# auduno/headtrackr

Measured on NVIDIA H100. Metric: frames/sec @640x480 (detect+CAMShift), higher is better.
Workload: dtype u8+f64

## Files before the change

headtrackr_b200/_lib.py:

```python
import ctypes as C
import os
import shutil
import subprocess
from pathlib import Path

_PKG = Path(__file__).resolve().parent
SO_PATH = Path(os.environ["HT_LIB"]).resolve() if os.environ.get("HT_LIB") else _PKG / "libheadtrackr_b200.so"
CSRC = _PKG / "csrc"

HT_OK, HT_WARN_OVERFLOW = 0, 1
HT_ERR_ARG, HT_ERR_CUDA, HT_ERR_SIZE, HT_ERR_CASCADE, HT_ERR_STATE = -1, -2, -3, -4, -5


class HtError(RuntimeError):
    def __init__(self, code, msg):
        super().__init__(f"headtrackr_b200 error {code}: {msg}")
        self.code = code


class Rect(C.Structure):
    _fields_ = [("x", C.c_double), ("y", C.c_double), ("width", C.c_double), ("height", C.c_double),
                ("confidence", C.c_double), ("neighbors", C.c_int32), ("pad_", C.c_int32)]


# ... 128 lines not shown
                ("cuda_stream", C.c_void_p)]


def sources_newer_than_so():
    if not SO_PATH.exists():
        return True
    t = SO_PATH.stat().st_mtime
    srcs = list(CSRC.glob("*.cu")) + list(CSRC.glob("*.cuh")) + list(CSRC.glob("*.inc")) + \
        [_PKG.parent / "include" / "headtrackr_b200.h"]
    return any(s.stat().st_mtime > t for s in srcs)


def nvcc():
    home = os.environ.get("CUDA_HOME") or os.environ.get("CUDA_PATH")
    if home and (Path(home) / "bin" / "nvcc").exists():
        return str(Path(home) / "bin" / "nvcc")
    return shutil.which("nvcc") or "/usr/local/cuda/bin/nvcc"


def build(force=False):
    if force or sources_newer_than_so():
        subprocess.check_call(["make", "-s", "-C", str(CSRC), f"NVCC={nvcc()}"] + (["-B"] if force else []))
    if not SO_PATH.exists():
        raise ImportError(f"{SO_PATH} was not produced by the build")
    return SO_PATH


_lib = None

EXPORTS = ["ht_version", "ht_create", "ht_destroy", "ht_last_error", "ht_sync", "ht_max_rects", "ht_detect",
           "ht_track_init", "ht_track_init_from_detect", "ht_track", "ht_detect_track", "ht_stream_reset", "ht_stream_step", "ht_stream_head_config", "ht_stream_step_head",
           "ht_tracker_config", "ht_tracker_reset", "ht_tracker_start", "ht_tracker_stop", "ht_tracker_step", "ht_tracker_feed", "ht_tracker_set_params", "ht_tracker_feed_canvases", "ht_tracker_set_debug", "ht_tracker_set_debug_strokes", "ht_tracker_set_face_crop", "ht_tracker_set_face_crop_yuv", "ht_tracker_set_face_tensor", "ht_face_crop_map", "ht_tracker_set_camera", "ht_tracker_export", "ht_tracker_import", "ht_tracker_feed_yuv", "ht_ingest", "ht_ingest_yuv",
           "ht_tracker_feed_views", "ht_tracker_feed_yuv_views", "ht_ingest_views", "ht_ingest_yuv_views", "ht_backprojection", "ht_whitebalance",
           "ht_plan_info", "ht_debug_plane", "ht_debug_raw", "ht_debug_model_hist", "ht_debug_track_stats", "ht_set_track_memo", "ht_set_pipeline", "ht_join", "ht_debug_set_exactness", "ht_debug_track_trace", "ht_debug_track_phases", "ht_launch_count",
           "ht_profile", "ht_profile_read"]

PROF_CLASSES = ["gray", "pyramid", "cascade", "group", "hist", "track_init", "track"]


def lib():
    global _lib
    if _lib is not None:
        return _lib
    if not SO_PATH.exists():
        try:
            build()
        except Exception as e:
            raise ImportError(f"libheadtrackr_b200.so is missing and could not be built: {e}") from e
    L = C.CDLL(str(SO_PATH))
    vp = C.c_void_p
    L.ht_version.restype = C.c_uint32
    L.ht_create.argtypes = [C.POINTER(vp), C.POINTER(Config), C.c_char_p, C.c_size_t]
    L.ht_destroy.argtypes = [vp]
    L.ht_destroy.restype = None
    L.ht_last_error.argtypes = [vp]
    L.ht_last_error.restype = C.c_char_p
    L.ht_sync.argtypes = [vp]
    L.ht_max_rects.argtypes = [vp]
    L.ht_detect.argtypes = [vp, vp, C.c_int, C.c_int, C.c_int, C.c_int, C.c_int, vp, vp]
    L.ht_track_init.argtypes = [vp, vp, C.c_int, vp, C.c_int, C.c_int, vp, C.c_int]
    L.ht_track_init_from_detect.argtypes = [vp, vp, C.c_int, vp, C.c_int, C.c_int, vp, vp, C.c_int, vp]
    L.ht_track.argtypes = [vp, vp, C.c_int, vp, C.c_int, C.c_int, C.c_int, vp, vp]
    L.ht_detect_track.argtypes = [vp, vp, C.c_int, C.c_int, C.c_int, C.c_int, C.c_int, C.c_int, C.c_int,
                                  vp, vp, vp, vp, vp]
    L.ht_stream_reset.argtypes = [vp, C.c_int, C.c_int]
    L.ht_stream_step.argtypes = [vp, vp, C.c_int, C.c_int, C.c_int, C.c_int, C.c_int, C.c_int, vp]
    L.ht_stream_head_config.argtypes = [vp, vp]
    L.ht_stream_step_head.argtypes = [vp, vp, C.c_int, C.c_int, C.c_int, C.c_int, C.c_int, C.c_int, vp, vp]
    L.ht_tracker_config.argtypes = [vp, vp]
    for f in (L.ht_tracker_reset, L.ht_tracker_start, L.ht_tracker_stop):
        f.argtypes = [vp, C.c_int, C.c_int]
    L.ht_tracker_step.argtypes = [vp, vp, C.c_int, C.c_int, C.c_int, C.c_double, vp]
    L.ht_tracker_feed.argtypes = [vp, vp, C.c_int, C.c_int, C.c_int, C.c_int, vp]
    L.ht_tracker_set_params.argtypes = [vp, C.c_int, C.c_int, vp]
    L.ht_tracker_feed_canvases.argtypes = [vp, vp, C.c_int, C.c_int, vp]
    L.ht_tracker_set_debug.argtypes = [vp, C.c_int, C.c_int, vp]
    L.ht_tracker_set_debug_strokes.argtypes = [vp, C.c_int, C.c_int, vp]
    L.ht_tracker_set_face_crop.argtypes = [vp, C.c_int, C.c_int, vp]
    L.ht_tracker_set_face_crop_yuv.argtypes = [vp, C.c_int, C.c_int, vp]
    L.ht_tracker_set_face_tensor.argtypes = [vp, C.c_int, C.c_int, vp]
    L.ht_face_crop_map.argtypes = [vp, C.c_int, C.c_int, C.c_int, C.c_int, vp, vp, vp]
    L.ht_tracker_set_camera.argtypes = [vp, C.c_int, C.c_int, vp]
    L.ht_tracker_export.argtypes = [vp, vp, C.c_int, vp]
    L.ht_tracker_import.argtypes = [vp, vp, C.c_int, vp]
    L.ht_ingest.argtypes = [vp, vp, C.c_int, C.c_int, C.c_int, vp, C.c_int, C.c_int]
    L.ht_tracker_feed_yuv.argtypes = [vp, vp, C.c_int, C.c_int, vp]
    L.ht_ingest_yuv.argtypes = [vp, vp, C.c_int, C.c_int, vp, C.c_int, C.c_int]
    L.ht_tracker_feed_views.argtypes = [vp, vp, vp, C.c_int, C.c_int, vp]
    L.ht_tracker_feed_yuv_views.argtypes = [vp, vp, vp, C.c_int, C.c_int, vp]
    L.ht_ingest_views.argtypes = [vp, vp, vp, C.c_int, C.c_int, vp, C.c_int, C.c_int]
    L.ht_ingest_yuv_views.argtypes = [vp, vp, vp, C.c_int, C.c_int, vp, C.c_int, C.c_int]
    L.ht_backprojection.argtypes = [vp, C.c_int, vp, C.c_int, C.c_int, vp]
    L.ht_whitebalance.argtypes = [vp, vp, C.c_int, C.c_int, C.c_int, vp]
    L.ht_plan_info.argtypes = [vp, C.c_int, C.c_int, C.c_int, vp, vp, vp, vp, C.c_int]
    L.ht_debug_plane.argtypes = [vp, C.c_int, C.c_int, C.c_int, vp, C.c_int, vp, vp]
    L.ht_debug_raw.argtypes = [vp, C.c_int, vp, C.c_int, vp]
    L.ht_debug_model_hist.argtypes = [vp, C.c_int, vp]
    L.ht_debug_track_stats.argtypes = [vp, vp, C.c_int]
    L.ht_debug_track_trace.argtypes = [vp, vp, C.c_int]
    L.ht_debug_track_phases.argtypes = [vp, vp, C.c_int]
    L.ht_set_track_memo.argtypes = [vp, C.c_int]
    L.ht_set_pipeline.argtypes = [vp, C.c_int]
    L.ht_join.argtypes = [vp]
    L.ht_debug_set_exactness.argtypes = [vp, C.c_int]
    L.ht_launch_count.argtypes = [vp]
    L.ht_launch_count.restype = C.c_uint64
    L.ht_profile.argtypes = [vp, C.c_int]
    L.ht_profile_read.argtypes = [vp, vp, vp, C.c_int]
    _lib = L
    return L
```

headtrackr_b200/context.py:

```python
import ctypes as C
import math

import numpy as np

from . import _lib
from ._lib import (Camera, CameraControl, CanvasFrame, DebugCanvas, FaceCrop, FaceCropYuv, FaceTensor, HeadEvent, HeadParams, HtError, Rect, StreamEvent, TrackerEvent, TrackerParams, TrackObj, VideoFrame,
                   VideoView, Window, YuvFrame, YuvImage)
from .views import video_view
from .synth import load_cascade_blob


def _is_torch(x):
    return hasattr(x, "data_ptr") and hasattr(x, "is_cuda")


def _frames_ptr(frames):
    if _is_torch(frames):
        t = frames
        if t.dim() == 3:
            t = t.unsqueeze(0)
        if not t.is_contiguous() or t.element_size() != 1 or t.shape[-1] != 4:
            raise ValueError("frames tensor must be contiguous uint8 (n,H,W,4)")
        return t.data_ptr(), t.shape[0], t.shape[1], t.shape[2], t
    a = np.ascontiguousarray(frames, dtype=np.uint8)
# ... 720 lines not shown
        cnt = C.c_int32()
        self._check(self._L.ht_debug_raw(self._h, frame, C.addressof(out), cap, C.addressof(cnt)))
        kept = min(cnt.value, cap, self.raw_cap)
        return [(r.x, r.y, r.width, r.height, r.confidence, r.neighbors) for r in out[:kept]], cnt.value

    def debug_track_stats(self, reset=True):
        out = (C.c_uint64 * 5)()
        self._check(self._L.ht_debug_track_stats(self._h, C.addressof(out), int(bool(reset))))
        return dict(passes=int(out[0]), serial_passes=int(out[1]), pixels=int(out[2]), calls=int(out[3]),
                    memo_hits=int(out[4]))

    def set_track_memo(self, enable=True):
        self._check(self._L.ht_set_track_memo(self._h, int(bool(enable))))

    def set_pipeline(self, enable=True):
        self._check(self._L.ht_set_pipeline(self._h, int(bool(enable))))

    def join(self):
        self._check(self._L.ht_join(self._h))

    def debug_set_exactness(self, flags):
        self._check(self._L.ht_debug_set_exactness(self._h, int(flags)))

    def debug_track_trace(self, n):
        out = np.zeros((n, 4), np.uint64)
        self._check(self._L.ht_debug_track_trace(self._h, out.ctypes.data, n))
        return out

    def debug_track_phases(self, n):
        out = np.zeros((n, 8), np.uint64)
        self._check(self._L.ht_debug_track_phases(self._h, out.ctypes.data, n))
        return out

    def debug_model_hist(self, slot):
        out = np.zeros(4096, np.uint32)
        self._check(self._L.ht_debug_model_hist(self._h, slot, out.ctypes.data))
        return out


def tracker_params(retryDetection=True, calcAngles=False, smoothing=True, fov=None, cameraOffset=11.5, headPosition=True,
                   edgecorrection=True, alpha=0.35, distance_to_screen=60.0):
    head = HeadParams(int(bool(smoothing)), int(bool(headPosition)), int(bool(edgecorrection)), 0, alpha,
                      float(fov) if fov is not None else 0.0, cameraOffset, distance_to_screen)
    return TrackerParams(int(bool(retryDetection)), int(bool(calcAngles)), (C.c_int32 * 2)(), head)


def tracker_event_dict(e):
    return dict(detection=("", "VJ", "CS", "WB")[e.detection], x=e.x, y=e.y, width=e.width, height=e.height,
                angle=e.angle, confidence=e.confidence, wb=e.wb, running=bool(e.running), fov=e.fov,
                status=[s for b, s in enumerate(_lib.TRACKER_STATUS) if e.status >> b & 1],
                head=dict(valid=bool(e.head.valid), x=e.head.x, y=e.head.y, z=e.head.z,
                          face=(e.head.fx, e.head.fy, e.head.fwidth, e.head.fheight)))


def tracker_events_from_bytes(buf):
    n = len(buf) // C.sizeof(TrackerEvent)
    arr = (TrackerEvent * n).from_buffer_copy(bytes(buf[: n * C.sizeof(TrackerEvent)]))
    return [tracker_event_dict(e) for e in arr]
```

headtrackr_b200/csrc/ht_api.cu:

```cuda
#include "../../include/headtrackr_b200.h"

#include <cuda.h>
#include <cuda_runtime.h>

#include <algorithm>
#include <cassert>
#include <cmath>
#include <cstdarg>
#include <cstddef>
#include <cstdio>
#include <cstdlib>
#include <cstring>
#include <map>
#include <memory>
#include <string>
#include <tuple>
#include <utility>
#include <vector>

#include "ht_common.cuh"
#include "ht_detect.cuh"
#include "ht_track.cuh"

using namespace ht;
// ... 320 lines not shown
    int g = 0;
    const int cuts_fast[] = {0, 2, 3, 4, 6};
    const int cuts_int[] = {0, 2, 4, 6};
    const int cuts_fp[] = {0, 2, 4, 6, 9};
    static_assert(HT_GEN_STAGES == 8, "cuts_fast assumes 8 generated stages");
    if (hc.fast) {
      for (int cpos : cuts_fast) cc.group_first[g++] = cpos;
      cc.group_first[g] = HT_GEN_STAGES;
      cc.late_int = 1;
    } else if (ints_ok && !getenv("HT_NO_LATE")) {
      for (int cpos : cuts_int) if (cpos < hc.n_stages) cc.group_first[g++] = cpos;
      cc.group_first[g] = std::min(8, hc.n_stages);
      cc.late_int = 1;
    } else {
      for (int cpos : cuts_fp) if (cpos < hc.n_stages) cc.group_first[g++] = cpos;
      cc.group_first[g] = hc.n_stages;
      cc.late_int = 0;
    }
    cc.n_groups = g;
  }
  hc.late.clear();
  hc.late_chunk0.assign((size_t)hc.n_stages + 1, 0);
  hc.late_conflicts = 0;
  for (int j = 0; j < hc.n_stages; ++j) {
    hc.late_chunk0[j] = (int32_t)(hc.late.size() / 32);
    if (j < cc.group_first[cc.n_groups]) continue;
    std::vector<int> rem;
    for (int k = cc.stage[j].first; k < cc.stage[j].first + cc.stage[j].count; ++k) rem.push_back(k);
    std::stable_sort(rem.begin(), rem.end(), [&](int x, int y) {
      const int sx = (cc.np_nn[x] & 15) + (cc.np_nn[x] >> 4), sy = (cc.np_nn[y] & 15) + (cc.np_nn[y] >> 4);
      return sx > sy;
    });
    while (!rem.empty()) {
      int bank_word[10][32];
      for (auto &row : bank_word) for (int &v : row) v = -1;
      auto place_side = [&](int k, int side, uint16_t *out, bool allow_conflicts, bool dry) -> int {
        const int cnt = side ? (cc.np_nn[k] >> 4) : (cc.np_nn[k] & 15);
        const uint16_t *pt = &cc.off[k][side ? 5 : 0];
        int order[5] = {0, 1, 2, 3, 4}, best_cost = 1 << 30, best[5] = {0, 1, 2, 3, 4};
        do {
          int cost = 0;
          for (int i = 0; i < cnt; ++i) {
            const int slot = side * 5 + order[i], word = pt[i] & 0x7fff, bw = bank_word[slot][word & 31];
            if (bw >= 0 && bw != word) cost += 1 << 10;
            cost += order[i];
          }
          if (cost < best_cost) { best_cost = cost; for (int i = 0; i < 5; ++i) best[i] = order[i]; }
        } while (std::next_permutation(order, order + 5));
        const int conflicts = best_cost >> 10;
        if (conflicts && !allow_conflicts) return -1;
        if (!dry) {
          for (int i = 0; i < cnt; ++i) {
            const int slot = side * 5 + best[i], word = pt[i] & 0x7fff;
            if (bank_word[slot][word & 31] < 0) bank_word[slot][word & 31] = word;
            out[slot] = pt[i];
          }
        }
        return conflicts;
      };
      for (int lane = 0; lane < 32; ++lane) {
        struct { uint16_t off[10]; int32_t a_int; } lf;
        for (int q = 0; q < 10; ++q) lf.off[q] = 0xFFFF;
        lf.a_int = 0;
        if (!rem.empty()) {
          size_t pick = rem.size();
          for (size_t i = 0; i < rem.size() && pick == rem.size(); ++i)
            if (place_side(rem[i], 0, lf.off, false, true) == 0 && place_side(rem[i], 1, lf.off, false, true) == 0) pick = i;
          if (pick == rem.size()) {
            int best_c = 1 << 30;
            for (size_t i = 0; i < rem.size(); ++i) {
              const int cfl = place_side(rem[i], 0, lf.off, true, true) + place_side(rem[i], 1, lf.off, true, true);
              if (cfl < best_c) { best_c = cfl; pick = i; }
            }
          }
          const int k = rem[pick];
          hc.late_conflicts += place_side(k, 0, lf.off, true, false) + place_side(k, 1, lf.off, true, false);
          lf.a_int = (int32_t)a_int[k];
          rem.erase(rem.begin() + (long)pick);
        }
        LateFeat rec{};
        for (int q = 0; q < 10; ++q) rec.off[q] = late_encode(lf.off[q]);
        rec.a_int = lf.a_int;
        hc.late.push_back(rec);
      }
    }
  }
  hc.late_chunk0[hc.n_stages] = (int32_t)(hc.late.size() / 32);
// ... 2672 lines not shown
int ht_join(ht_ctx *ctx) {
  if (!ctx) return HT_ERR_ARG;
  return join_aux(ctx);
}

int ht_debug_track_stats(ht_ctx *ctx, uint64_t *out5, int reset) {
  if (!ctx || !out5) return HT_ERR_ARG;
  CK(cudaSetDevice(ctx->cfg.device));
  CK(cudaStreamSynchronize(ctx->stream));
  CK(cudaMemcpy(out5, ctx->d_flags.as<unsigned long long>() + 8, 5 * sizeof(uint64_t), cudaMemcpyDeviceToHost));
  if (reset) CK(cudaMemset(ctx->d_flags.as<unsigned long long>() + 8, 0, 5 * sizeof(uint64_t)));
  return HT_OK;
}

int ht_debug_track_trace(ht_ctx *ctx, uint64_t *out, int n) {
  if (!ctx || !out) return HT_ERR_ARG;
  if (!ctx->track_trace || !ctx->d_trace.p || n < 0 || n > ctx->cfg.max_frames)
    return ctx->fail(HT_ERR_ARG, "track timeline is not enabled (HT_TRACK_TRACE=1 at ht_create) or n is out of range");
  CK(cudaSetDevice(ctx->cfg.device));
  CK(cudaStreamSynchronize(ctx->stream));
  CK(cudaMemcpy(out, ctx->d_trace.p, 4 * sizeof(uint64_t) * (size_t)n, cudaMemcpyDeviceToHost));
  return HT_OK;
}

int ht_debug_track_phases(ht_ctx *ctx, uint64_t *out, int n) {
  if (!ctx) return HT_ERR_ARG;
  { const int jr = join_aux(ctx); if (jr != HT_OK) return jr; }
  if (!ctx->track_trace || !ctx->d_trace.p || n < 0 || n > ctx->cfg.max_frames)
    return ctx->fail(HT_ERR_ARG, "no track trace (create the context with HT_TRACK_TRACE=1)");
  CK(cudaSetDevice(ctx->cfg.device));
  CK(cudaStreamSynchronize(ctx->stream));
  CK(cudaMemcpy(out, ctx->d_trace.as<unsigned long long>() + 4 * (size_t)ctx->cfg.max_frames, 8 * sizeof(uint64_t) * (size_t)n, cudaMemcpyDeviceToHost));
  return HT_OK;
}

int ht_debug_model_hist(ht_ctx *ctx, int slot, uint32_t *out4096) {
  if (!ctx) return HT_ERR_ARG;
  { const int jr = join_aux(ctx); if (jr != HT_OK) return jr; }
  if (!out4096 || slot < 0 || slot >= ctx->cfg.max_frames || !ctx->model_hist.p) return ctx->fail(HT_ERR_ARG, "bad slot");
  CK(cudaSetDevice(ctx->cfg.device));
  CK(cudaStreamSynchronize(ctx->stream));
  CK(cudaMemcpy(out4096, ctx->model_hist.as<uint32_t>() + (size_t)slot * 4096, 4096 * sizeof(uint32_t), cudaMemcpyDeviceToHost));
  return HT_OK;
}

}

#ifdef HT_HOST_SELFTEST
extern "C" int ht_selftest_planes(int w, int h, int interval, int32_t *out, int cap) {
  Plan P;
  std::string err;
  if (build_plan(P, w, h, interval, 24, 24, err, false) != HT_OK) return -1;
  if ((int)P.planes.size() * 6 + 2 > cap) return -2;
  out[0] = (int32_t)P.planes.size();
  out[1] = (int32_t)P.arena_stride;
  for (size_t i = 0; i < P.planes.size(); ++i) {
    int slot = -1, q = -1;
    for (size_t k = 0; k < P.plane_id.size(); ++k) if (P.plane_id[k] == (int)i) { slot = (int)(k / 4); q = (int)(k % 4); }
    int32_t *o = out + 2 + 6 * i;
    o[0] = (int32_t)P.planes[i].off; o[1] = P.planes[i].pitch; o[2] = P.planes[i].w; o[3] = P.planes[i].h; o[4] = slot; o[5] = q;
  }
  return 0;
}

extern "C" int ht_selftest_head(const ht_head_params *params, int n, const double *cs , int camw,
                                int camh, ht_head_event *out) {
// ... 504 lines not shown
      }
  }
  for (int f = 0; f < 4; ++f) {
    std::sort(hits[f].begin(), hits[f].end(), [](const Hit &a, const Hit &b) { return a.key < b.key; });
    counts[f] = (int32_t)hits[f].size();
    for (size_t i = 0; i < hits[f].size() && (int)i < cap; ++i) {
      double *o = out + ((size_t)f * cap + i) * 4;
      o[0] = hits[f][i].x; o[1] = hits[f][i].y; o[2] = hits[f][i].width; o[3] = hits[f][i].conf;
    }
  }
  return 0;
}

int main(int argc, char **argv) {
  if (argc < 2) { fprintf(stderr, "usage: %s cascade.bin\n", argv[0]); return 2; }
  FILE *f = fopen(argv[1], "rb");
  if (!f) { perror("open"); return 2; }
  std::vector<uint8_t> blob;
  uint8_t buf[4096];
  size_t got;
  while ((got = fread(buf, 1, sizeof(buf), f)) > 0) blob.insert(blob.end(), buf, buf + got);
  fclose(f);
  HostCascade hc;
  std::string err;
  const int rc = parse_cascade(blob.data(), blob.size(), hc, err);
  if (rc != HT_OK) { fprintf(stderr, "parse_cascade: %s\n", err.c_str()); return 1; }
  const ConstCascade &cc = hc.cc;
  const int late_first = cc.group_first[cc.n_groups];
  long long bad = 0, used_slots = 0, used_instr = 0, conflicts = 0;
  for (int j = late_first; j < hc.n_stages; ++j) {
    std::vector<int> seen((size_t)cc.stage[j].count, 0);
    for (int ch = hc.late_chunk0[j]; ch < hc.late_chunk0[j + 1]; ++ch) {
      for (int s = 0; s < 10; ++s) {
        int bank_word[32];
        for (int &v : bank_word) v = -1;
        bool any = false;
        for (int lane = 0; lane < 32; ++lane) {
          const uint16_t o = late_decode(hc.late[(size_t)ch * 32 + lane].off[s]);
          if (o == 0xFFFF) continue;
          any = true; ++used_slots;
          const int word = o & 0x7fff;
          if (bank_word[word & 31] >= 0 && bank_word[word & 31] != word) ++conflicts;
          bank_word[word & 31] = word;
        }
        used_instr += any ? 1 : 0;
      }
      for (int lane = 0; lane < 32; ++lane) {
        const LateFeat &lf = hc.late[(size_t)ch * 32 + lane];
        std::vector<uint16_t> p, n;
        for (int s = 0; s < 5; ++s) if (lf.off[s] != LATE_UNUSED) p.push_back(late_decode(lf.off[s]));
        for (int s = 5; s < 10; ++s) if (lf.off[s] != LATE_UNUSED) n.push_back(late_decode(lf.off[s]));
        if (p.empty() && n.empty()) { if (lf.a_int != 0) ++bad; continue; }
        std::sort(p.begin(), p.end()); std::sort(n.begin(), n.end());
        int match = -1;
        for (int k = cc.stage[j].first; k < cc.stage[j].first + cc.stage[j].count && match < 0; ++k) {
          if (seen[(size_t)(k - cc.stage[j].first)]) continue;
          std::vector<uint16_t> kp(cc.off[k], cc.off[k] + (cc.np_nn[k] & 15)), kn(cc.off[k] + 5, cc.off[k] + 5 + (cc.np_nn[k] >> 4));
          std::sort(kp.begin(), kp.end()); std::sort(kn.begin(), kn.end());
          if (kp == p && kn == n && llround(cc.alpha[k] * 1e8) == lf.a_int) match = k;
        }
        if (match < 0) ++bad; else seen[(size_t)(match - cc.stage[j].first)] = 1;
      }
    }
    for (int v : seen) if (!v) ++bad;
  }
  printf("{\"n_stages\": %d, \"n_features\": %d, \"fast\": %d, \"n_groups\": %d, \"late_first\": %d, \"chunks\": %d, "
         "\"bad\": %lld, \"point_loads\": %lld, \"load_instr_with_traffic\": %lld, \"bank_conflicts\": %lld, \"late_conflicts\": %d}\n",
         hc.n_stages, hc.n_features, hc.fast ? 1 : 0, cc.n_groups, late_first, hc.late_chunk0[hc.n_stages], bad, used_slots,
         used_instr, conflicts, hc.late_conflicts);
  return bad ? 1 : 0;
}
#endif
```

headtrackr_b200/csrc/ht_common.cuh:

```cuda
#pragma once
#include <cstddef>
#include <cstdint>

namespace ht {

constexpr int TW = 32;
constexpr int TH = 8;
constexpr int NV = 2 * TH;
constexpr int L0_COLS = 4 * TW + 22;
constexpr int L0_ROWS = 4 * TH + 22;
constexpr int H0 = L0_COLS / 2;
constexpr int P0 = L0_COLS;
constexpr int L1_ROWS = 2 * TH + 11;
constexpr int L1_COLS = 2 * TW + 11;
constexpr int P1 = 76;
constexpr int L2_ROWS = TH + 5;
constexpr int L2_COLS = TW + 5;
constexpr int P2 = 76;
constexpr int W1 = (L0_ROWS * P0 + 31) / 32 * 32;
constexpr int W2 = W1 + L1_ROWS * P1;
constexpr int TILE_WORDS = W2 + 2 * L2_ROWS * P2;
__host__ __device__ constexpr int tile_l0(int r, int X) { return r * P0 + (X & 1) * H0 + (X >> 1); }
__host__ __device__ constexpr int tile_l1(int r, int c) { return W1 + r * P1 + c; }
__host__ __device__ constexpr int tile_l2(int rr, int c2) { return W2 + rr * P2 + c2; }
constexpr int VA = 2 * P0;
constexpr int VB = P1;
static_assert((VA - VB) % 32 == 0 && P1 == P2, "bank classes of the two bases must coincide");
static_assert(2 * L2_COLS <= P2 && L1_COLS <= P1, "tile pitches");
constexpr int BANK_K = VA % 32;
static_assert(VB % 32 == BANK_K, "bank_class");
constexpr int NWIN = TW * TH * 4 * 4;
constexpr int MASK_WORDS = NV / 4;
static_assert(NV % 4 == 0, "TH must be even");
constexpr int CASCADE_THREADS = 256;
constexpr int CASCADE_WARPS = CASCADE_THREADS / 32;
__host__ __device__ constexpr int point_word(int z, int x, int y) {
  return z == 0 ? tile_l0(y, x) : z == 1 ? tile_l1(y, x) : tile_l2(2 * y, 2 * x);
}
__host__ __device__ constexpr int bank_class(int u, int v) { return (u + BANK_K * v) & 31; }
__host__ __device__ constexpr int class_u(int c, int v, int uh) { return ((c - BANK_K * v) & 31) + 32 * uh; }

constexpr int MAX_STAGES = 64;
constexpr int MAX_GROUPS = 16;

struct DevPlane {
  uint32_t off;
  int32_t pitch;
  int32_t w, h;
};

struct alignas(16) DevJob {
  uint32_t src_off, dst_off;
  int32_t src_pitch, dst_pitch;
  int32_t dst_h;
  int32_t dw, dh;
  uint32_t col_off;
  uint32_t row_off;
  uint32_t magic, shift;
// ... 86 lines not shown
```

headtrackr_b200/csrc/ht_detect.cuh:

```cuda
#pragma once
#include "ht_common.cuh"

namespace ht {

__host__ __device__ __forceinline__ unsigned quad_frames(int quad, int n_frames, const uint8_t *__restrict__ quad_mask) {
  const int left = n_frames - 4 * quad;
  const unsigned prefix = left >= 4 ? 15u : (left > 0 ? (1u << left) - 1u : 0u);
  return quad_mask ? (prefix & quad_mask[quad]) : prefix;
}

__host__ __device__ __forceinline__ uint32_t rgb_bin(uint32_t px) {
  return ((px & 0xf0u) << 4) | ((px >> 8) & 0xf0u) | ((px >> 20) & 0xfu);
}

__host__ __device__ __forceinline__ uint32_t gray_of(uint32_t px) {
#ifdef __CUDA_ARCH__
  const double M = 4503599627370496.0;
  const double r = __dsub_rn(__hiloint2double(0x43300000, (int)__byte_perm(px, 0u, 0x4440)), M);
  const double g = __dsub_rn(__hiloint2double(0x43300000, (int)__byte_perm(px, 0u, 0x4441)), M);
  const double b = __dsub_rn(__hiloint2double(0x43300000, (int)__byte_perm(px, 0u, 0x4442)), M);
  const double v = __dadd_rn(__dadd_rn(__dmul_rn(r, 0.3), __dmul_rn(g, 0.59)), __dmul_rn(b, 0.11));
  const uint32_t iv = (uint32_t)__double2loint(__dadd_rn(v, M));
  return min(iv, 255u);
#else
// ... 787 lines not shown
}

template <int V>
struct IntC {
  __host__ __device__ constexpr operator int() const { return V; }
};
__device__ __forceinline__ int warp_max_i32(int v) { return (int)__reduce_max_sync(0xffffffffu, (unsigned)v); }
__device__ __forceinline__ long long warp_sum_i64(long long v) {
  const unsigned long long u = (unsigned long long)(v + (1ll << 46));
  const unsigned lo = __reduce_add_sync(0xffffffffu, (unsigned)(u & 0xffffffull));
  const unsigned hi = __reduce_add_sync(0xffffffffu, (unsigned)(u >> 24));
  return (long long)(((unsigned long long)hi << 24) + lo) - (32ll << 46);
}
__device__ __forceinline__ int nth_bit32(uint32_t w, int r) {
  int pos = 0, t;
  t = __popc(w & 0xffffu); if (r >= t) { r -= t; pos += 16; w >>= 16; }
  t = __popc(w & 0xffu);   if (r >= t) { r -= t; pos += 8;  w >>= 8; }
  t = __popc(w & 0xfu);    if (r >= t) { r -= t; pos += 4;  w >>= 4; }
  t = __popc(w & 0x3u);    if (r >= t) { r -= t; pos += 2;  w >>= 2; }
  t = (int)(w & 1u);       if (r >= t) pos += 1;
  return pos;
}
__device__ __forceinline__ int nth_set_bit(const uint32_t *__restrict__ masks, int c, int r) {
#pragma unroll
  for (int j = 0; j < MASK_WORDS; ++j) {
    const uint32_t w = masks[j * 32 + c];
    const int pc = __popc(w);
    if (r < pc) return j * 32 + nth_bit32(w, r);
    r -= pc;
  }
  return -1;
}

template <bool FAST>
__global__ void __launch_bounds__(CASCADE_THREADS, 4) k_cascade(DevPlan plan, const LateFeat *__restrict__ late,
                                                                const LateFeat *__restrict__ feat_orig,
                                                                const int32_t *__restrict__ late_chunk0,
                                                                const void *__restrict__ tmaps, int tma_quad0,
                                                                const uint32_t *__restrict__ arena, size_t quad_stride,
                                                                int n_frames, uint32_t *__restrict__ raw_keys,
                                                                double *__restrict__ raw_conf,
                                                                uint32_t *__restrict__ raw_count, int raw_cap,
                                                                int force_ties, const uint8_t *__restrict__ quad_mask) {
  if (quad_frames(blockIdx.y, n_frames, quad_mask) == 0u) return;
  extern __shared__ __align__(128) uint32_t smem[];
  uint32_t *tile = smem;
  uint32_t *masks = smem + TILE_WORDS;
  __shared__ __align__(8) unsigned long long tma_bar;

  const int tid = threadIdx.x, lane = tid & 31, warp = tid >> 5;
  const int quad = blockIdx.y;
  const DevCascTile tl = plan.casc_tiles[blockIdx.x];
  const DevScale sc = plan.scales[tl.scale];
  const uint32_t *qa = arena + (size_t)quad * quad_stride;
  const int x0 = tl.tx * TW, y0 = tl.ty * TH;
  const unsigned fmask = quad_frames(quad, n_frames, quad_mask);

  for (int i = tid; i < 3 * MASK_WORDS * 32; i += CASCADE_THREADS) masks[i] = 0u;

  const bool use_tma = tmaps != nullptr;
  if (use_tma) {
    const unsigned bar = (unsigned)__cvta_generic_to_shared(&tma_bar);
    if (tid == 0) {
      asm volatile("mbarrier.init.shared::cta.b64 [%0], 1;" ::"r"(bar));
      asm volatile("fence.mbarrier_init.release.cluster;" ::: "memory");
    }
    __syncthreads();
    if (tid == 0) {
      asm volatile("mbarrier.arrive.expect_tx.shared::cta.b64 _, [%0], %1;" ::"r"(bar), "r"((unsigned)(L1_ROWS * P1 * 4)) : "memory");
      const unsigned dst = (unsigned)__cvta_generic_to_shared(tile + W1);
      const unsigned long long map = (unsigned long long)(reinterpret_cast<const uint8_t *>(tmaps) + 128 * (size_t)tl.scale);
      asm volatile(
          "cp.async.bulk.tensor.3d.shared::cluster.global.tile.mbarrier::complete_tx::bytes [%0], [%1, {%2, %3, %4}], [%5];"
          ::"r"(dst), "l"(map), "r"(2 * x0), "r"(2 * y0), "r"(tma_quad0 + quad), "r"(bar)
          : "memory");
    }
  }
  {
    {
      const DevPlane pl = plan.planes[sc.p0];
      const uint32_t *src = qa + pl.off;
      const int X0 = 4 * x0, Y0 = 4 * y0;
      constexpr int G0 = (L0_COLS + 3) / 4;
      for (int i0 = tid; i0 < L0_ROWS * G0; i0 += 4 * CASCADE_THREADS) {
        uint4 v[4];
#pragma unroll
        for (int k = 0; k < 4; ++k) {
          const int i = i0 + k * CASCADE_THREADS, r = i / G0, X = (i - r * G0) * 4;
          v[k] = make_uint4(0u, 0u, 0u, 0u);
          if (i < L0_ROWS * G0 && Y0 + r < pl.h && X0 + X < pl.pitch)
            v[k] = __ldg(reinterpret_cast<const uint4 *>(src + (size_t)(Y0 + r) * pl.pitch + X0 + X));
        }
#pragma unroll
        for (int k = 0; k < 4; ++k) {
          const int i = i0 + k * CASCADE_THREADS, r = i / G0, X = (i - r * G0) * 4;
          if (i >= L0_ROWS * G0) break;
          uint32_t *row = tile + tile_l0(r, X);
          if (X + 2 < L0_COLS) *reinterpret_cast<uint2 *>(row) = make_uint2(v[k].x, v[k].z);
          else row[0] = v[k].x;
          if (X + 1 < L0_COLS) row[H0] = v[k].y;
          if (X + 3 < L0_COLS) row[H0 + 1] = v[k].w;
        }
      }
    }
    if (!use_tma) {
      const DevPlane pl = plan.planes[sc.p1];
      const uint32_t *src = qa + pl.off;
      const int X0 = 2 * x0, Y0 = 2 * y0;
      constexpr int G1 = P1 / 4;
      for (int i = tid; i < L1_ROWS * G1; i += CASCADE_THREADS) {
        const int r = i / G1, c = (i - r * G1) * 4;
        const bool ok = (Y0 + r < pl.h) && (X0 + c < pl.pitch);
        const unsigned dst = (unsigned)__cvta_generic_to_shared(tile + tile_l1(r, c));
        asm volatile("cp.async.cg.shared.global [%0], [%1], 16, %2;" ::"r"(dst), "l"(ok ? src + (size_t)(Y0 + r) * pl.pitch + X0 + c : src),
                     "r"(ok ? 16u : 0u) : "memory");
      }
    }
    {
      constexpr int G2 = (L2_COLS + 3) / 4;
      for (int i = tid; i < 2 * L2_ROWS * G2; i += CASCADE_THREADS) {
        const int dy = i / (L2_ROWS * G2), rem = i - dy * (L2_ROWS * G2), r = rem / G2, c = (rem - r * G2) * 4;
        uint4 v0 = make_uint4(0u, 0u, 0u, 0u), v1 = v0;
        {
          const DevPlane pl = plan.planes[plan.scales[tl.scale].p2[2 * dy]];
          if (y0 + r < pl.h && x0 + c < pl.pitch) v0 = __ldg(reinterpret_cast<const uint4 *>(qa + pl.off + (size_t)(y0 + r) * pl.pitch + x0 + c));
        }
        {
          const DevPlane pl = plan.planes[plan.scales[tl.scale].p2[2 * dy + 1]];
          if (y0 + r < pl.h && x0 + c < pl.pitch) v1 = __ldg(reinterpret_cast<const uint4 *>(qa + pl.off + (size_t)(y0 + r) * pl.pitch + x0 + c));
        }
        uint32_t *row = tile + tile_l2(2 * r + dy, 2 * c);
        *reinterpret_cast<uint4 *>(row) = make_uint4(v0.x, v1.x, v0.y, v1.y);
        if (2 * c + 8 <= P2) *reinterpret_cast<uint4 *>(row + 4) = make_uint4(v0.z, v1.z, v0.w, v1.w);
      }
    }
    asm volatile("cp.async.commit_group;\n\tcp.async.wait_group 0;" ::: "memory");
  }
  if (use_tma) {
    const unsigned bar = (unsigned)__cvta_generic_to_shared(&tma_bar);
    unsigned done = 0;
    for (int spin = 0; !done && spin < (1 << 24); ++spin) {
      asm volatile("{\n\t.reg .pred p;\n\tmbarrier.try_wait.parity.shared::cta.b64 p, [%1], 0;\n\tselp.u32 %0, 1, 0, p;\n\t}"
                   : "=r"(done) : "r"(bar) : "memory");
    }
    if (!done) __trap();
  }
  __syncthreads();

  const uint8_t *tile_b = reinterpret_cast<const uint8_t *>(tile);
  auto emit = [&](int c, int b, double sum) {
    const int v = b >> 3, uh = (b >> 2) & 1, f = b & 3, u = class_u(c, v, uh);
    const int lx = u >> 1, ly = v >> 1, q = (u & 1) | ((v & 1) << 1);
    const uint32_t key = sc.win_base + (uint32_t)((q * sc.qh + (y0 + ly)) * sc.qw + (x0 + lx));
    const int frame = 4 * quad + f;
    const uint32_t pos = atomicAdd(&raw_count[frame], 1u);
    if (pos < (uint32_t)raw_cap) {
      raw_keys[(size_t)frame * raw_cap + pos] = key;
      raw_conf[(size_t)frame * raw_cap + pos] = sum;
    }
  };
  auto bases = [&](int c, int b, const uint8_t *&tA, const uint8_t *&tB) {
    const int v = b >> 3, uh = (b >> 2) & 1, f = b & 3, u = class_u(c, v, uh);
    tA = tile_b + 4 * (v * VA + u) + f;
    tB = tile_b + 4 * (v * VB + u) + f;
  };
  const int late_first = c_casc.group_first[c_casc.n_groups];
  const bool has_late = late_first < c_casc.n_stages;
  uint32_t *m_in = masks, *m_out = masks + MASK_WORDS * 32, *m_clr = masks + 2 * MASK_WORDS * 32;
  int g = 0;

  {
    constexpr int NQ = HT_QUAD_STAGES < HT_GEN_QUAD_STAGES ? HT_QUAD_STAGES : HT_GEN_QUAD_STAGES;
    static_assert(NQ == 2 || NQ == 3, "the dense group is {0,1} or {0,1,2}");
    uint16_t *m16 = reinterpret_cast<uint16_t *>(m_in);
    for (int chunk = warp; chunk < NV / 2; chunk += CASCADE_WARPS) {
      uint32_t bits = 0;
#pragma unroll 1
      for (int unit = 0; unit < 4; ++unit) {
        const int v = 2 * chunk + (unit >> 1), uh = unit & 1, u = class_u(lane, v, uh);
        const int lx = u >> 1, ly = v >> 1;
// ... 17 lines not shown
        if (tt & bit) {                                                                                      \
          const uint8_t *bA = reinterpret_cast<const uint8_t *>(tA) + f, *bB = reinterpret_cast<const uint8_t *>(tB) + f; \
          if (!stage_pass_ordered(bA, bB, J)) pp &= ~bit;                                                    \
        }                                                                                                    \
      }                                                                                                      \
    }                                                                                                        \
    a_lo &= p_lo; a_hi &= p_hi;                                                                              \
  }
          HT_QSTAGE(0)
          HT_QSTAGE(1)
#if HT_GEN_QUAD_STAGES >= 3
          HT_QSTAGE(2)
#endif
#undef HT_QSTAGE
          m = ((a_lo >> 15) & 1u) | ((a_hi >> 14) & 2u) | ((a_lo >> 29) & 4u) | ((a_hi >> 28) & 8u);
        } else {
          for (int f = 0; f < 4; ++f) {
            bool alive = (x0 + lx < sc.qw) && (y0 + ly < sc.qh) && ((fmask >> f) & 1u);
            const uint8_t *tA = tile_b + 4 * (v * VA + u) + f, *tB = tile_b + 4 * (v * VB + u) + f;
            for (int j = c_casc.group_first[0]; j < c_casc.group_first[1]; ++j) {
              if (!__any_sync(0xffffffffu, alive)) break;
              alive = alive && stage_pass_ordered(tA, tB, j);
            }
            m |= (alive ? 1u : 0u) << f;
          }
        }
        bits |= m << (4 * unit);
      }
      m16[(((chunk >> 1) * 32 + lane) << 1) | (chunk & 1)] = (uint16_t)bits;
    }
    g = FAST ? (NQ >= 3 ? 2 : 1) : 1;
  }
  __syncthreads();

  auto run_group = [&](auto JB, auto JE, const bool emit_here) __attribute__((always_inline)) -> bool {
    const int jb = JB, je = JE;
    int n = 0;
#pragma unroll
    for (int j = 0; j < MASK_WORDS; ++j) n += __popc(m_in[j * 32 + lane]);
    if (warp_max_i32(n) == 0) return true;
    for (int i = tid; i < MASK_WORDS * 32; i += CASCADE_THREADS) m_clr[i] = 0u;
    const int r_beg = (warp * n) / CASCADE_WARPS, r_end = ((warp + 1) * n) / CASCADE_WARPS;
    const int my_iters = r_end - r_beg;
    const int iters = warp_max_i32(my_iters);
    int bpos = my_iters > 0 ? nth_set_bit(m_in, lane, r_beg) : 0;
    uint32_t cur = my_iters > 0 ? (m_in[(bpos >> 5) * 32 + lane] & (0xffffffffu << (bpos & 31))) : 0u;
    for (int it = 0; it < iters; ++it) {
      bool alive = it < my_iters;
      int b = 0;
      if (alive) {
        while (cur == 0u) { bpos = (bpos | 31) + 1; cur = m_in[(bpos >> 5) * 32 + lane]; }
        b = (bpos & ~31) | (__ffs(cur) - 1);
        cur &= cur - 1u;
        bpos = b;
      }
      const uint8_t *tA, *tB;
      bases(lane, b, tA, tB);
      double sum = 0.0;
#pragma unroll
      for (int j = jb; j < je; ++j) {
        if (!__any_sync(0xffffffffu, alive)) break;
        if (FAST && j < HT_GEN_STAGES) {
          int rr = gen_stage(j, tA, tB);
          if (force_ties & 1) rr = -1;
          if (rr < 0) rr = stage_pass_ordered(tA, tB, j) ? 1 : 0;
          alive = alive && (rr != 0);
        } else {
          sum = stage_sum_ordered(tA, tB, j);
          alive = alive && !(sum < c_casc.stage[j].threshold);
        }
      }
      if (alive) {
        if (emit_here) {
          if (FAST && je - 1 < HT_GEN_STAGES) sum = stage_sum_ordered(tA, tB, je - 1);
          emit(lane, b, sum);
        } else {
          atomicOr(&m_out[(b >> 5) * 32 + lane], 1u << (b & 31));
        }
      }
    }
    if (emit_here) return true;
    __syncthreads();
    uint32_t *t = m_in; m_in = m_out; m_out = m_clr; m_clr = t;
    return false;
  };
  if (FAST) {
    static_assert(HT_GEN_STAGES == 8, "compile-time groups assume 8 generated stages");
    if (g < 2 && run_group(IntC<2>{}, IntC<3>{}, false)) return;
    if (run_group(IntC<3>{}, IntC<4>{}, false)) return;
    if (run_group(IntC<4>{}, IntC<6>{}, false)) return;
    if (run_group(IntC<6>{}, IntC<8>{}, !has_late)) return;
  } else {
    for (; g < c_casc.n_groups; ++g)
      if (run_group(c_casc.group_first[g], c_casc.group_first[g + 1], (g == c_casc.n_groups - 1) && !has_late)) return;
  }
  if (!has_late) {
    if (c_casc.n_groups == 1) {
      int n = 0;
#pragma unroll
      for (int j = 0; j < MASK_WORDS; ++j) n += __popc(m_in[j * 32 + lane]);
      for (int r = warp; r < n; r += CASCADE_WARPS) {
        const int b = nth_set_bit(m_in, lane, r);
        const uint8_t *tA, *tB;
        bases(lane, b, tA, tB);
        emit(lane, b, stage_sum_ordered(tA, tB, c_casc.n_stages - 1));
      }
    }
    return;
  }

  {
    int mylen = 0;
#pragma unroll
    for (int j = 0; j < MASK_WORDS; ++j) mylen += __popc(m_in[j * 32 + lane]);
    int incl = mylen;
#pragma unroll
    for (int o = 1; o < 32; o <<= 1) {
      const int t = __shfl_up_sync(0xffffffffu, incl, o);
      if (lane >= o) incl += t;
    }
    const int total = __shfl_sync(0xffffffffu, incl, 31), excl = incl - mylen;
    for (int wdx = warp; wdx < total; wdx += CASCADE_WARPS) {
      const unsigned owner = __ballot_sync(0xffffffffu, wdx >= excl && wdx < incl);
      const int c = __ffs(owner) - 1;
      const int b = nth_set_bit(m_in, c, wdx - __shfl_sync(0xffffffffu, excl, c));
      const uint8_t *tA, *tB;
      bases(c, b, tA, tB);
      const unsigned sA = (unsigned)__cvta_generic_to_shared(tA), sBm = (unsigned)__cvta_generic_to_shared(tB) - 0x80000000u;
// ... 202 lines not shown
```

include/headtrackr_b200.h:

```cpp
#ifndef HEADTRACKR_B200_H
#define HEADTRACKR_B200_H

#include <stddef.h>
#include <stdint.h>

#ifdef __cplusplus
extern "C" {
#endif

#define HT_OK 0
#define HT_WARN_OVERFLOW 1
#define HT_ERR_ARG (-1)
#define HT_ERR_CUDA (-2)
#define HT_ERR_SIZE (-3)
#define HT_ERR_CASCADE (-4)
#define HT_ERR_STATE (-5)

typedef struct ht_ctx ht_ctx;

typedef struct {
  double x, y, width, height, confidence;
  int32_t neighbors;
  int32_t pad_;
} ht_rect;
// ... 242 lines not shown
  double scaling;
  double fixed_position[3];
  double look_at[3];
  double screen_height, damping;
  double fov, aspect, near, far;
} ht_camera_control;
int ht_tracker_set_camera(ht_ctx *ctx, int first, int n, const ht_camera_control *controls);

#define HT_TRACKER_RECORD_BYTES 16864
#define HT_TRACKER_RECORD_MAGIC 0x31525448u
#define HT_TRACKER_RECORD_VERSION 1u
int ht_tracker_export(ht_ctx *ctx, const int32_t *streams, int n, void *records);
int ht_tracker_import(ht_ctx *ctx, const int32_t *streams, int n, const void *records);

int ht_ingest(ht_ctx *ctx, const uint8_t *src_rgba, int n, int sw, int sh, uint8_t *dst_rgba, int dw, int dh);

int ht_backprojection(ht_ctx *ctx, int slot, const uint8_t *rgba, int w, int h, uint8_t *out_rgba);

int ht_whitebalance(ht_ctx *ctx, const uint8_t *rgba, int n, int w, int h, double *out);


int ht_plan_info(ht_ctx *ctx, int w, int h, int interval, int32_t *n_slots, int32_t *scale_upto,
                 int32_t *slot_w, int32_t *slot_h, int cap);
int ht_debug_plane(ht_ctx *ctx, int frame, int slot, int q, uint8_t *out, int cap_bytes, int32_t *w, int32_t *h);
int ht_debug_raw(ht_ctx *ctx, int frame, ht_rect *out, int cap, int32_t *count);
int ht_debug_model_hist(ht_ctx *ctx, int slot, uint32_t *out4096);
int ht_debug_track_stats(ht_ctx *ctx, uint64_t *out5, int reset);
int ht_debug_set_exactness(ht_ctx *ctx, int flags);
int ht_set_track_memo(ht_ctx *ctx, int enable);
int ht_set_pipeline(ht_ctx *ctx, int enable);
int ht_join(ht_ctx *ctx);
int ht_debug_track_trace(ht_ctx *ctx, uint64_t *out, int n_streams);
int ht_debug_track_phases(ht_ctx *ctx, uint64_t *out, int n_streams);
uint64_t ht_launch_count(const ht_ctx *ctx);

enum { HT_PROF_GRAY = 0, HT_PROF_PYRAMID, HT_PROF_CASCADE, HT_PROF_GROUP, HT_PROF_HIST, HT_PROF_TRACK_INIT,
       HT_PROF_TRACK, HT_PROF_N };
int ht_profile(ht_ctx *ctx, int enable);
int ht_profile_read(ht_ctx *ctx, double *ms_out, uint64_t *launches_out, int reset);

#ifdef __cplusplus
}
#endif
#endif
```

Before: 76580.

## Split level-0 tile into separate even/odd planes with 16-byte stores; widen pitches

Changes the shared-memory layout of the level-0 tile so even and odd columns live in two separate planes (OB offset) with a pitch of 76, and raises the level-1/2 pitches to 88. The tile load now reads two uint4 per item and writes two full uint4 rows instead of scattered 2- and 1-word stores, which cuts shared store instructions and bank conflicts during tile fill. The host-side feature placement and conflict accounting are updated to track multiple words per bank, because the new layout can map several words to the same bank class. Also adds an optional compile-time clock64 phase trace for k_cascade with an API to read it. The tile grows in shared memory, which may lower occupancy, and the changed bank mapping could make cascade feature reads conflict more.

Result: no change. 77180 (median of 6 runs) (+0.8%).

```diff
diff --git a/headtrackr_b200/_lib.py b/headtrackr_b200/_lib.py
--- a/headtrackr_b200/_lib.py
+++ b/headtrackr_b200/_lib.py
@@ -184,7 +184,7 @@
            "ht_track_init", "ht_track_init_from_detect", "ht_track", "ht_detect_track", "ht_stream_reset", "ht_stream_step", "ht_stream_head_config", "ht_stream_step_head",
            "ht_tracker_config", "ht_tracker_reset", "ht_tracker_start", "ht_tracker_stop", "ht_tracker_step", "ht_tracker_feed", "ht_tracker_set_params", "ht_tracker_feed_canvases", "ht_tracker_set_debug", "ht_tracker_set_debug_strokes", "ht_tracker_set_face_crop", "ht_tracker_set_face_crop_yuv", "ht_tracker_set_face_tensor", "ht_face_crop_map", "ht_tracker_set_camera", "ht_tracker_export", "ht_tracker_import", "ht_tracker_feed_yuv", "ht_ingest", "ht_ingest_yuv",
            "ht_tracker_feed_views", "ht_tracker_feed_yuv_views", "ht_ingest_views", "ht_ingest_yuv_views", "ht_backprojection", "ht_whitebalance",
-           "ht_plan_info", "ht_debug_plane", "ht_debug_raw", "ht_debug_model_hist", "ht_debug_track_stats", "ht_set_track_memo", "ht_set_pipeline", "ht_join", "ht_debug_set_exactness", "ht_debug_track_trace", "ht_debug_track_phases", "ht_launch_count",
+           "ht_plan_info", "ht_debug_plane", "ht_debug_raw", "ht_debug_model_hist", "ht_debug_track_stats", "ht_set_track_memo", "ht_set_pipeline", "ht_join", "ht_debug_set_exactness", "ht_debug_track_trace", "ht_debug_track_phases", "ht_debug_cascade_phases", "ht_launch_count",
            "ht_profile", "ht_profile_read"]
 
 PROF_CLASSES = ["gray", "pyramid", "cascade", "group", "hist", "track_init", "track"]
@@ -251,6 +251,7 @@
     L.ht_debug_track_stats.argtypes = [vp, vp, C.c_int]
     L.ht_debug_track_trace.argtypes = [vp, vp, C.c_int]
     L.ht_debug_track_phases.argtypes = [vp, vp, C.c_int]
+    L.ht_debug_cascade_phases.argtypes = [vp, vp, C.c_int]
     L.ht_set_track_memo.argtypes = [vp, C.c_int]
     L.ht_set_pipeline.argtypes = [vp, C.c_int]
     L.ht_join.argtypes = [vp]
diff --git a/headtrackr_b200/context.py b/headtrackr_b200/context.py
--- a/headtrackr_b200/context.py
+++ b/headtrackr_b200/context.py
@@ -776,6 +776,11 @@
         self._check(self._L.ht_debug_track_phases(self._h, out.ctypes.data, n))
         return out
 
+    def debug_cascade_phases(self, reset=False):
+        out = np.zeros(8, np.uint64)
+        self._check(self._L.ht_debug_cascade_phases(self._h, out.ctypes.data, int(bool(reset))))
+        return out
+
     def debug_model_hist(self, slot):
         out = np.zeros(4096, np.uint32)
         self._check(self._L.ht_debug_model_hist(self._h, slot, out.ctypes.data))
diff --git a/headtrackr_b200/csrc/ht_api.cu b/headtrackr_b200/csrc/ht_api.cu
--- a/headtrackr_b200/csrc/ht_api.cu
+++ b/headtrackr_b200/csrc/ht_api.cu
@@ -376,8 +376,11 @@
       return sx > sy;
     });
     while (!rem.empty()) {
-      int bank_word[10][32];
-      for (auto &row : bank_word) for (int &v : row) v = -1;
+      std::vector<int> bank_words[10][32];
+      auto conflicts_with = [&](int slot, int word) {
+        const std::vector<int> &v = bank_words[slot][word & 31];
+        return !v.empty() && std::find(v.begin(), v.end(), word) == v.end();
+      };
       auto place_side = [&](int k, int side, uint16_t *out, bool allow_conflicts, bool dry) -> int {
         const int cnt = side ? (cc.np_nn[k] >> 4) : (cc.np_nn[k] & 15);
         const uint16_t *pt = &cc.off[k][side ? 5 : 0];
@@ -385,8 +388,8 @@
         do {
           int cost = 0;
           for (int i = 0; i < cnt; ++i) {
-            const int slot = side * 5 + order[i], word = pt[i] & 0x7fff, bw = bank_word[slot][word & 31];
-            if (bw >= 0 && bw != word) cost += 1 << 10;
+            const int slot = side * 5 + order[i], word = pt[i] & 0x7fff;
+            if (conflicts_with(slot, word)) cost += 1 << 10;
             cost += order[i];
           }
           if (cost < best_cost) { best_cost = cost; for (int i = 0; i < 5; ++i) best[i] = order[i]; }
@@ -396,7 +399,8 @@
         if (!dry) {
           for (int i = 0; i < cnt; ++i) {
             const int slot = side * 5 + best[i], word = pt[i] & 0x7fff;
-            if (bank_word[slot][word & 31] < 0) bank_word[slot][word & 31] = word;
+            std::vector<int> &v = bank_words[slot][word & 31];
+            if (std::find(v.begin(), v.end(), word) == v.end()) v.push_back(word);
             out[slot] = pt[i];
           }
         }
@@ -3135,6 +3139,24 @@
   CK(cudaStreamSynchronize(ctx->stream));
   CK(cudaMemcpy(out, ctx->d_trace.as<unsigned long long>() + 4 * (size_t)ctx->cfg.max_frames, 8 * sizeof(uint64_t) * (size_t)n, cudaMemcpyDeviceToHost));
   return HT_OK;
+}
+
+int ht_debug_cascade_phases(ht_ctx *ctx, uint64_t *out8, int reset) {
+  if (!ctx) return HT_ERR_ARG;
+#if HT_CASCADE_PHASETRACE
+  { const int jr = join_aux(ctx); if (jr != HT_OK) return jr; }
+  CK(cudaSetDevice(ctx->cfg.device));
+  CK(cudaStreamSynchronize(ctx->stream));
+  if (out8) CK(cudaMemcpyFromSymbol(out8, g_casc_phases, 8 * sizeof(uint64_t)));
+  if (reset) {
+    const unsigned long long zero[8] = {};
+    CK(cudaMemcpyToSymbol(g_casc_phases, zero, sizeof(zero)));
+  }
+  return HT_OK;
+#else
+  (void)out8; (void)reset;
+  return ctx->fail(HT_ERR_ARG, "k_cascade phase totals need a profiling build (-DHT_CASCADE_PHASETRACE=1)");
+#endif
 }
 
 int ht_debug_model_hist(ht_ctx *ctx, int slot, uint32_t *out4096) {
@@ -3705,16 +3727,18 @@
     std::vector<int> seen((size_t)cc.stage[j].count, 0);
     for (int ch = hc.late_chunk0[j]; ch < hc.late_chunk0[j + 1]; ++ch) {
       for (int s = 0; s < 10; ++s) {
-        int bank_word[32];
-        for (int &v : bank_word) v = -1;
+        std::vector<int> bank_words[32];
         bool any = false;
         for (int lane = 0; lane < 32; ++lane) {
           const uint16_t o = late_decode(hc.late[(size_t)ch * 32 + lane].off[s]);
           if (o == 0xFFFF) continue;
           any = true; ++used_slots;
           const int word = o & 0x7fff;
-          if (bank_word[word & 31] >= 0 && bank_word[word & 31] != word) ++conflicts;
-          bank_word[word & 31] = word;
+          std::vector<int> &v = bank_words[word & 31];
+          if (std::find(v.begin(), v.end(), word) == v.end()) {
+            if (!v.empty()) ++conflicts;
+            v.push_back(word);
+          }
         }
         used_instr += any ? 1 : 0;
       }
diff --git a/headtrackr_b200/csrc/ht_common.cuh b/headtrackr_b200/csrc/ht_common.cuh
--- a/headtrackr_b200/csrc/ht_common.cuh
+++ b/headtrackr_b200/csrc/ht_common.cuh
@@ -9,21 +9,22 @@
 constexpr int NV = 2 * TH;
 constexpr int L0_COLS = 4 * TW + 22;
 constexpr int L0_ROWS = 4 * TH + 22;
-constexpr int H0 = L0_COLS / 2;
-constexpr int P0 = L0_COLS;
+constexpr int PE = 76;
+constexpr int OB = (L0_ROWS * PE + 31) / 32 * 32;
 constexpr int L1_ROWS = 2 * TH + 11;
 constexpr int L1_COLS = 2 * TW + 11;
-constexpr int P1 = 76;
+constexpr int P1 = 88;
 constexpr int L2_ROWS = TH + 5;
 constexpr int L2_COLS = TW + 5;
-constexpr int P2 = 76;
-constexpr int W1 = (L0_ROWS * P0 + 31) / 32 * 32;
+constexpr int P2 = 88;
+constexpr int W1 = 2 * OB;
 constexpr int W2 = W1 + L1_ROWS * P1;
 constexpr int TILE_WORDS = W2 + 2 * L2_ROWS * P2;
-__host__ __device__ constexpr int tile_l0(int r, int X) { return r * P0 + (X & 1) * H0 + (X >> 1); }
+static_assert(2 * PE >= L0_COLS && PE % 4 == 0 && P1 % 4 == 0 && OB % 4 == 0 && W1 % 32 == 0, "16-byte rows, level 1 128-byte aligned");
+__host__ __device__ constexpr int tile_l0(int r, int X) { return (X & 1) * OB + r * PE + (X >> 1); }
 __host__ __device__ constexpr int tile_l1(int r, int c) { return W1 + r * P1 + c; }
 __host__ __device__ constexpr int tile_l2(int rr, int c2) { return W2 + rr * P2 + c2; }
-constexpr int VA = 2 * P0;
+constexpr int VA = 2 * PE;
 constexpr int VB = P1;
 static_assert((VA - VB) % 32 == 0 && P1 == P2, "bank classes of the two bases must coincide");
 static_assert(2 * L2_COLS <= P2 && L1_COLS <= P1, "tile pitches");
diff --git a/headtrackr_b200/csrc/ht_detect.cuh b/headtrackr_b200/csrc/ht_detect.cuh
--- a/headtrackr_b200/csrc/ht_detect.cuh
+++ b/headtrackr_b200/csrc/ht_detect.cuh
@@ -843,6 +843,34 @@
   return -1;
 }
 
+#ifndef HT_CASCADE_PHASETRACE
+#define HT_CASCADE_PHASETRACE 0
+#endif
+#if HT_CASCADE_PHASETRACE
+__device__ unsigned long long g_casc_phases[8];
+struct CascPhaseTrace {
+  bool on;
+  long long t[5];
+  __device__ explicit CascPhaseTrace(bool on_) : on(on_), t{0, 0, 0, 0, 0} { mark(0); }
+  __device__ void mark(int i) { if (on) t[i] = clock64(); }
+  __device__ ~CascPhaseTrace() {
+    if (!on) return;
+    const long long end = clock64();
+    const long long e2 = t[2] ? t[2] : end, e3 = t[3] ? t[3] : end, e4 = t[4] ? t[4] : end;
+    atomicAdd(&g_casc_phases[0], (unsigned long long)(e2 - t[0]));
+    atomicAdd(&g_casc_phases[1], (unsigned long long)(e3 - e2));
+    atomicAdd(&g_casc_phases[2], (unsigned long long)(e4 - e3));
+    atomicAdd(&g_casc_phases[3], (unsigned long long)(end - e4));
+    atomicAdd(&g_casc_phases[4], 1ull);
+    if (t[1]) atomicAdd(&g_casc_phases[5], (unsigned long long)(e2 - t[1]));
+    if (t[4]) atomicAdd(&g_casc_phases[6], 1ull);
+  }
+};
+#define HT_CP_MARK(i) ptrace.mark(i)
+#else
+#define HT_CP_MARK(i) do { } while (0)
+#endif
+
 template <bool FAST>
 __global__ void __launch_bounds__(CASCADE_THREADS, 4) k_cascade(DevPlan plan, const LateFeat *__restrict__ late,
                                                                 const LateFeat *__restrict__ feat_orig,
@@ -854,6 +882,9 @@
                                                                 uint32_t *__restrict__ raw_count, int raw_cap,
                                                                 int force_ties, const uint8_t *__restrict__ quad_mask) {
   if (quad_frames(blockIdx.y, n_frames, quad_mask) == 0u) return;
+#if HT_CASCADE_PHASETRACE
+  CascPhaseTrace ptrace(threadIdx.x == 0);
+#endif
   extern __shared__ __align__(128) uint32_t smem[];
   uint32_t *tile = smem;
   uint32_t *masks = smem + TILE_WORDS;
@@ -892,25 +923,25 @@
       const DevPlane pl = plan.planes[sc.p0];
       const uint32_t *src = qa + pl.off;
       const int X0 = 4 * x0, Y0 = 4 * y0;
-      constexpr int G0 = (L0_COLS + 3) / 4;
-      for (int i0 = tid; i0 < L0_ROWS * G0; i0 += 4 * CASCADE_THREADS) {
-        uint4 v[4];
-#pragma unroll
-        for (int k = 0; k < 4; ++k) {
-          const int i = i0 + k * CASCADE_THREADS, r = i / G0, X = (i - r * G0) * 4;
-          v[k] = make_uint4(0u, 0u, 0u, 0u);
-          if (i < L0_ROWS * G0 && Y0 + r < pl.h && X0 + X < pl.pitch)
-            v[k] = __ldg(reinterpret_cast<const uint4 *>(src + (size_t)(Y0 + r) * pl.pitch + X0 + X));
+      constexpr int G0 = 2 * PE / 8;
+      for (int i0 = tid; i0 < L0_ROWS * G0; i0 += 2 * CASCADE_THREADS) {
+        uint4 v[2][2];
+#pragma unroll
+        for (int k = 0; k < 2; ++k) {
+          const int i = i0 + k * CASCADE_THREADS, r = i / G0, X = (i - r * G0) * 8;
+          v[k][0] = v[k][1] = make_uint4(0u, 0u, 0u, 0u);
+          if (i < L0_ROWS * G0 && Y0 + r < pl.h) {
+            const uint4 *g = reinterpret_cast<const uint4 *>(src + (size_t)(Y0 + r) * pl.pitch + X0 + X);
+            if (X0 + X < pl.pitch) v[k][0] = __ldg(g);
+            if (X0 + X + 4 < pl.pitch) v[k][1] = __ldg(g + 1);
+          }
         }
 #pragma unroll
-        for (int k = 0; k < 4; ++k) {
-          const int i = i0 + k * CASCADE_THREADS, r = i / G0, X = (i - r * G0) * 4;
+        for (int k = 0; k < 2; ++k) {
+          const int i = i0 + k * CASCADE_THREADS, r = i / G0, X = (i - r * G0) * 8;
           if (i >= L0_ROWS * G0) break;
-          uint32_t *row = tile + tile_l0(r, X);
-          if (X + 2 < L0_COLS) *reinterpret_cast<uint2 *>(row) = make_uint2(v[k].x, v[k].z);
-          else row[0] = v[k].x;
-          if (X + 1 < L0_COLS) row[H0] = v[k].y;
-          if (X + 3 < L0_COLS) row[H0 + 1] = v[k].w;
+          *reinterpret_cast<uint4 *>(tile + tile_l0(r, X)) = make_uint4(v[k][0].x, v[k][0].z, v[k][1].x, v[k][1].z);
+          *reinterpret_cast<uint4 *>(tile + tile_l0(r, X + 1)) = make_uint4(v[k][0].y, v[k][0].w, v[k][1].y, v[k][1].w);
         }
       }
     }
@@ -942,11 +973,12 @@
         }
         uint32_t *row = tile + tile_l2(2 * r + dy, 2 * c);
         *reinterpret_cast<uint4 *>(row) = make_uint4(v0.x, v1.x, v0.y, v1.y);
-        if (2 * c + 8 <= P2) *reinterpret_cast<uint4 *>(row + 4) = make_uint4(v0.z, v1.z, v0.w, v1.w);
+        *reinterpret_cast<uint4 *>(row + 4) = make_uint4(v0.z, v1.z, v0.w, v1.w);
       }
     }
     asm volatile("cp.async.commit_group;\n\tcp.async.wait_group 0;" ::: "memory");
   }
+  HT_CP_MARK(1);
   if (use_tma) {
     const unsigned bar = (unsigned)__cvta_generic_to_shared(&tma_bar);
     unsigned done = 0;
@@ -957,6 +989,7 @@
     if (!done) __trap();
   }
   __syncthreads();
+  HT_CP_MARK(2);
 
   const uint8_t *tile_b = reinterpret_cast<const uint8_t *>(tile);
   auto emit = [&](int c, int b, double sum) {
@@ -1040,6 +1073,7 @@
     g = FAST ? (NQ >= 3 ? 2 : 1) : 1;
   }
   __syncthreads();
+  HT_CP_MARK(3);
 
   auto run_group = [&](auto JB, auto JE, const bool emit_here) __attribute__((always_inline)) -> bool {
     const int jb = JB, je = JE;
@@ -1102,6 +1136,7 @@
     for (; g < c_casc.n_groups; ++g)
       if (run_group(c_casc.group_first[g], c_casc.group_first[g + 1], (g == c_casc.n_groups - 1) && !has_late)) return;
   }
+  HT_CP_MARK(4);
   if (!has_late) {
     if (c_casc.n_groups == 1) {
       int n = 0;
diff --git a/include/headtrackr_b200.h b/include/headtrackr_b200.h
--- a/include/headtrackr_b200.h
+++ b/include/headtrackr_b200.h
@@ -298,6 +298,7 @@
 int ht_join(ht_ctx *ctx);
 int ht_debug_track_trace(ht_ctx *ctx, uint64_t *out, int n_streams);
 int ht_debug_track_phases(ht_ctx *ctx, uint64_t *out, int n_streams);
+int ht_debug_cascade_phases(ht_ctx *ctx, uint64_t *out8, int reset);
 uint64_t ht_launch_count(const ht_ctx *ctx);
 
 enum { HT_PROF_GRAY = 0, HT_PROF_PYRAMID, HT_PROF_CASCADE, HT_PROF_GROUP, HT_PROF_HIST, HT_PROF_TRACK_INIT,
```
